# sthagen/foundationdb

Hardware: AMD Instinct MI355X
Metric: resolved txns/sec (conflict ranges checked/sec) per batch; HBM GB/s vs peak (higher is better)
Workload: dtype u8/int64 (byte keys, int64 versions)

## Files before the change

### foundationdb_amd/csrc/engine.cpp

```cpp
#include <hip/hip_runtime.h>
#include <stdio.h>
#include <stdlib.h>
#include <string.h>
#include <unistd.h>

#include <cxxabi.h>

#include <algorithm>
#include <array>
#include <atomic>
#include <chrono>
#include <condition_variable>
#include <functional>
#include <mutex>
#include <new>
#include <string>
#include <thread>
#include <unordered_set>
#include <vector>

#include "../../include/fdb_conflict_set.h"
#include "engine.h"

using namespace fdbcs;
// ... 482 lines not shown
    for (int pass = 0; pass < 2; pass++) {
    if (pass == 1) {
        if (int rc = cs->ws[k][0].ensure(align_up(off, (size_t)2 << 20))) return rc;
        arena = (char*)cs->ws[k][0].p;
        off = 0;
    }
#define TAKE(field, bytes) \
    if (int rc = take((bytes), (void**)&w.field)) return rc
    TAKE(hist_conf, T);
    TAKE(rconf, R);
    TAKE(status, T);
    TAKE(first_conf, 4 * T);
    const int64_t slab_buckets = std::min<int64_t>(kSortMaxBuckets, (E + kSortTarget - 1) / kSortTarget + 1);
    TAKE(items, sizeof(SortItem) * E);
    TAKE(scnt, 8 * kCntStride * (size_t)kSortMaxBuckets);
    TAKE(slab, sizeof(SortItem) * kSlab * slab_buckets);
    TAKE(ovf, sizeof(SortItem) * E);
    TAKE(ovf_b, 4 * E);
    TAKE(big, sizeof(SortItem) * E);
    TAKE(big_p, 4 * E);
    TAKE(samples, sizeof(SortItem) * kMaxSample);
    TAKE(srank, 4 * (kMaxSample + 64));
    w.slab_buckets = (int32_t)slab_buckets;
    TAKE(pos, 4 * E);
    TAKE(pmeta, 4 * E);
    TAKE(cwb, 4 * (E + 1));
    TAKE(crb, 4 * (E + 1));
    TAKE(cwe, 4 * (E + 1));
    TAKE(wends, 8 * (2 * W + 1));
    TAKE(wkeys, sizeof(DKey) * (2 * W + 1));
    TAKE(segk, sizeof(DKey) * (2 * W + 2));
    TAKE(cflag, 2 * W + 2);
    TAKE(wbrange, 4 * W);
    TAKE(wlead, 4 * (W + 1));
    TAKE(wtxn, 4 * (W + 1));
    TAKE(gminc, 4 * (W + 1));
    TAKE(rbrange, 4 * R);
    TAKE(eoff, 4 * (R + 1));
    TAKE(poff, 4 * (R + W + 1));
    TAKE(pcg, 4 * (R + W + 1));
    TAKE(pcoff, 4 * (R + W + 1));
    TAKE(pcbase, 4 * (R + W + 1));
    TAKE(pca, 4 * (R + W + 1));
    TAKE(ecur, 4 * R);
    TAKE(edges, 4 * edge_cap);
    TAKE(eptr, 4 * T);
    TAKE(pre_st, T);
    TAKE(pre_ep, 4 * T);
    TAKE(pre_end, 4 * T);
    TAKE(ulist, 32 * T);
    TAKE(wpk, 4 * (W + 1));
    TAKE(tedges, 4 * edge_cap);
    TAKE(mcs_bits, 8 * (E / 64 + 2));
    TAKE(seg_b, 4 * (W + 1));
    TAKE(seg_e, 4 * (W + 1));
    TAKE(seg_lo, 8 * (W + 1));
    TAKE(seg_hi, 8 * (W + 1));
    TAKE(seg_rem, 8 * (W + 1));
    TAKE(seg_ins, 8 * (W + 1));
    TAKE(seg_tlen, 8 * (W + 1));
    TAKE(seg_endins, W + 1);
    TAKE(seg_vend, 8 * (W + 1));
    TAKE(verdict, T);
    TAKE(bsc, sizeof(BatchScalars));
    }
#undef TAKE
    w.edge_cap = edge_cap;
    w.cap_T = T;
    w.cap_R = R;
    HIPOK(hipMemsetAsync(w.hist_conf, 0, T, cs->stream));
    HIPOK(hipMemsetAsync(w.rconf, 0, R, cs->stream));
    HIPOK(hipMemsetAsync(w.ecur, 0, 4 * R, cs->stream));
    HIPOK(hipMemsetAsync(w.scnt, 0, 8 * kCntStride * (size_t)kSortMaxBuckets, cs->stream));
    HIPOK(hipMemsetAsync(w.srank, 0, 4 * (kMaxSample + 64), cs->stream));
    HIPOK(hipMemsetAsync(w.bsc, 0, sizeof(BatchScalars), cs->stream));
    if (k >= 1) {
        Work& w0 = cs->work[0];
        w.c_lo = w0.c_lo, w.c_hi = w0.c_hi, w.c_rem = w0.c_rem, w.c_ins = w0.c_ins, w.c_val = w0.c_val;
// ... 3079 lines not shown
```

### foundationdb_amd/csrc/engine.h

```cpp
#pragma once
#include <hip/hip_runtime.h>
#include <stdint.h>
#include <limits.h>

#include "dkey.h"
#include "scan.h"

namespace fdbcs {

constexpr int kBlock = 256;
constexpr int kWG = 1024;
constexpr int kSortTile = 4096;
constexpr int kFan = 64;
constexpr int kMaxLevels = 4;
constexpr int kL3Rep = 8;
constexpr int kL3Pad = 16;
__host__ __device__ constexpr int64_t l3_words(int64_t n) { return n * kL3Rep * kL3Pad; }
constexpr int kGcTile = 4096;
constexpr int kMaxGroupWrites = 12288;
constexpr int kMaxTxnLds = 49152;

enum : uint8_t { kUndecided = 0, kAborted = 1, kCommitted = 2 };
enum : uint8_t { kFlagTooOld = 1, kFlagReport = 2 };

// ... 60 lines not shown
    int32_t debug_error;
    int32_t ovf_n;
    int32_t sort_big;
    int64_t n_segments;
    int64_t n_pranges;
    int32_t n_undec;
    int32_t pad2;
};

constexpr int64_t kHole = INT64_MIN;

struct TierIO {
    const int64_t* n_in;
    int64_t* n_out;
    int64_t* before;
    int64_t* removed;
};

struct Segs {
    int64_t *lo, *hi, *rem, *ins;
    int32_t* tile_first;
};

enum ScanKind { kScanEdges, kScanSegSum, kScanCompact, kScanGc, kScanCover, kScanSegNum, kScanFold, kNumScans };

struct BatchDev {
    int32_t T, R, W;
    int64_t* snap;
    uint8_t* flags;
    int32_t* roff;
    int32_t* woff;
    int32_t* rowner;
    int32_t* wowner;
    DKey* keys;
    uint8_t* tail;
    int64_t tail_n;
};

#ifndef FDBCS_SORT_TARGET
#define FDBCS_SORT_TARGET 64
#endif
constexpr int kSortTarget = FDBCS_SORT_TARGET;
constexpr int kSlab = 256;
constexpr int kSortMaxBuckets = 4096;
constexpr int kQuant = 4096;
constexpr int kQuantMinE = 2048;
constexpr int kMaxSample = 8192;
// ... 3 lines not shown
constexpr int kCntStride = FDBCS_CNT_STRIDE;
constexpr int kSplitWords = 8;
constexpr int kSplitBytes = 8 * kSplitWords;
struct SplitKey {
    uint64_t w[kSplitWords];
    uint32_t len, meta;
};

struct Work {
    uint8_t* hist_conf;
    uint8_t* rconf;
    uint8_t* status;
    int32_t* first_conf;
    SortItem* items;
    uint64_t* scnt;
    SortItem* slab;
    int32_t slab_buckets;
    SortItem* ovf;
    int32_t* ovf_b;
    SortItem* big;
    int32_t* big_p;
    SortItem* samples;
    int32_t* srank;
    int32_t* pos;
    uint32_t* pmeta;
    int32_t* cwb;
    int32_t* crb;
    int32_t* cwe;
    int2* wends;
    DKey* wkeys;
    DKey* segk;
    uint8_t* cflag;
    uint8_t* btail;
    int32_t* wbrange;
    int32_t* rbrange;
    int32_t* eoff;
    int32_t* poff;
    int32_t* pcg;
    int32_t* pcoff;
    int32_t* pcbase;
    int32_t* pca;
    int32_t* ecur;
    int32_t* wlead;
    int32_t* wtxn;
    int32_t* gminc;
    int32_t groups = 0;
    int32_t* edges;
    int64_t edge_cap;
    int32_t* eptr;
    uint8_t* pre_st;
    int32_t* pre_ep;
    int32_t* pre_end;
    int4* ulist;
    uint32_t* wpk;
    int32_t report = 0;
    int32_t* tedges;
    uint64_t* mcs_bits;
    int32_t* seg_b;
    int32_t* seg_e;
    int64_t* seg_lo;
    int64_t* seg_hi;
    int64_t* seg_rem;
    int64_t* seg_ins;
    int64_t* seg_tlen;
    uint8_t* seg_endins;
    int64_t* seg_vend;
    uint8_t* verdict;
    BatchScalars* bsc;
    ScanState scan[kNumScans];
    int64_t scan_gran[kNumScans];
    uint64_t* scan_arena;
    int64_t scan_words;
    int64_t cap_T, cap_R;
    int32_t* tile_first;
    int64_t *c_lo, *c_hi, *c_rem, *c_ins, *c_val;
    uint8_t* c_exact;
    unsigned long long* trace;
    int32_t no_prepass;
    uint32_t* hedge;
    uint32_t hseq;
    uint8_t* vdev;
};
// ... 270 lines not shown
```

### foundationdb_amd/csrc/kernels.hip

```cpp
#include <hip/hip_runtime.h>
#include <stdio.h>
#include <stdlib.h>
#include <algorithm>
#include <vector>
#include <limits.h>

#include "engine.h"
#include "lane_xor.h"

namespace fdbcs {

thread_local LaunchList* t_record = nullptr;
thread_local uint8_t t_group = 0;
thread_local hipError_t t_launch_error = hipSuccess;


__device__ __forceinline__ const uint8_t* hist_tail(const uint8_t* htail, uint32_t unit) {
    return htail + 8 * (size_t)unit;
}
__device__ __forceinline__ uint32_t tail_units(uint32_t len) { return len > 16u ? (len - 16u + 7u) / 8u : 0u; }

__device__ __forceinline__ void copy_tail_words(uint8_t* dst, const uint8_t* src, uint32_t n) {
    const uintptr_t a = (uintptr_t)src;
    const uint64_t* w = (const uint64_t*)(a & ~(uintptr_t)7);
// ... 1215 lines not shown
    const uint32_t slot = (uint32_t)old;
    if (slot < (uint32_t)kSlab) {
        a.slab[(size_t)bk * kSlab + slot] = it;
    } else {
        const int o = atomicAdd(&a.bsc->ovf_n, 1);
        a.ovf[o] = it;
        a.ovf_b[o] = bk;
    }
    if (a.trace) {
        asm volatile("s_waitcnt vmcnt(0)" ::: "memory");
        trace_max(a.trace, kTrPartEnd);
        if ((threadIdx.x & 63) == 0) {
            const unsigned long long tp4 = wall_clock64();
            atomicAdd(&a.trace[kTrPartWaves], 1ull);
            atomicAdd(&a.trace[kTrPartSumFill], tp1 - tp0);
            atomicAdd(&a.trace[kTrPartSumCopy], tp2 - tp1);
            atomicAdd(&a.trace[kTrPartSumSearch], tp3 - tp2);
            atomicAdd(&a.trace[kTrPartSumPlace], tp4 - tp3);
        }
    }
}

struct SortOut {
    int32_t* pos;
    uint32_t* pmeta;
    int32_t *cwb, *crb, *cwe;
    int32_t *wbrange, *rbrange;
    SortItem* items;
    SplitKey* quant;
    SortItem* big;
    int32_t* big_p;
};

template <int S>
__device__ __forceinline__ void wave_bitonic(uint64_t (&kh)[4], uint64_t (&kl)[4], uint64_t (&ka)[4]) {
    const int lane = threadIdx.x & 63;
#pragma unroll
    for (int k = 2; k <= 64 * S; k <<= 1) {
#pragma unroll
        for (int j = k >> 1; j > 0; j >>= 1) {
            if (j >= 64) {
                const int js = j >> 6;
#pragma unroll
                for (int s = 0; s < S; s++) {
                    if (s & js) continue;
                    const int t = s | js;
                    const bool up = ((s * 64 + lane) & k) == 0;
                    if (key3_less(kh[t], kl[t], ka[t], kh[s], kl[s], ka[s]) == up) {
                        uint64_t x = kh[s]; kh[s] = kh[t]; kh[t] = x;
// ... 18 lines not shown
        }
    }
}

__device__ __forceinline__ uint32_t endpoint_meta(const BatchDev& b, int p) {
    const int g = p >> 1, e = p & 1;
    const uint32_t cls = g < b.R ? (e ? kReadEnd : kReadBegin) : (e ? kWriteEnd : kWriteBegin);
    return ((uint32_t)g << 3) | ((uint32_t)e << 2) | cls;
}

__device__ __forceinline__ void put_quantiles(const BatchDev& b, SplitKey* quant, int64_t P, int64_t E, int p) {
    int q = (int)((P * (kQuant + 1) + E - 1) / E) - 1;
    if (q < 0) q = 0;
    if (q >= kQuant || quant_pos(q, E) > P) return;
    const SplitKey sk = make_split(make_item(b, p), b.tail);
    for (; q < kQuant && quant_pos(q, E) <= P; q++)
        if (quant_pos(q, E) == P) quant[q] = sk;
}

__device__ __forceinline__ void put_position(const BatchDev& b, const SortOut& o, int p, int64_t P, int32_t wb,
                                             int32_t rb, int32_t we) {
    const uint32_t meta = endpoint_meta(b, p);
    const uint32_t cls = item_class(meta);
    o.pmeta[P] = meta;
    o.pos[p] = (int32_t)P;
    o.cwb[P] = wb;
    o.crb[P] = rb;
    o.cwe[P] = we;
    if (cls == kWriteBegin) o.wbrange[wb] = p >> 1;
    if (cls == kReadBegin) o.rbrange[rb] = p >> 1;
    if (o.items) o.items[P] = make_item(b, p);
}

__device__ __forceinline__ uint32_t split_lcp(const SplitKey& a, const SplitKey& b) {
    uint32_t c = 0;
#pragma unroll
    for (int i = 0; i < kSplitWords; i++) {
        const uint64_t x = a.w[i] ^ b.w[i];
        if (x) {
            c = 8 * i + (uint32_t)(__builtin_clzll(x) >> 3);
            break;
        }
        c = 8 * (i + 1);
    }
    c = c < a.len ? c : a.len;
    return c < b.len ? c : b.len;
}

template <bool LONG>
__global__ __launch_bounds__(kBlock) void k_sort_bucket(BatchDev b, SortArgs a, SortOut o) {
    constexpr int kWaves = kBlock / 64;
// ... 262 lines not shown
        if (lane == 0) {
#pragma unroll
            for (int c = 0; c < 4; c++) {
                s_red[c][wave] = pre[c];
                s_red[4 + c][wave] = tot[c];
            }
            const uint32_t v[4] = {(uint32_t)own0, (uint32_t)(own0 >> 32), (uint32_t)own1, (uint32_t)(own1 >> 32)};
#pragma unroll
            for (int c = 0; c < 4; c++) s_cnt[wave][c] = v[c];
            s_big[wave] = n > kSlab ? 1 : 0;
        }
        __syncthreads();
        if (threadIdx.x == 0) {
            uint32_t run[4] = {0, 0, 0, 0};
            for (int q = 0; q < kWaves; q++)
#pragma unroll
                for (int c = 0; c < 4; c++) run[c] += s_red[c][q];
            for (int q = 0; q < kWaves; q++)
#pragma unroll
                for (int c = 0; c < 4; c++) {
                    s_base[q][c] = run[c];
                    run[c] += s_cnt[q][c];
                }
            if (blockIdx.x == 0) {
                uint32_t t4[4] = {0, 0, 0, 0};
                for (int q = 0; q < kWaves; q++)
#pragma unroll
                    for (int c = 0; c < 4; c++) t4[c] += s_red[4 + c][q];
                o.cwb[E] = (int32_t)t4[1];
                o.crb[E] = (int32_t)t4[2];
                o.cwe[E] = (int32_t)t4[3];
            }
        }
        __syncthreads();
        if (threadIdx.x == 0) trace_max(a.trace, kTrBktPrologue);
    }
    if (small) {
        const int64_t base = s_base[wave][0];
        const unsigned long long tw3 = a.trace ? wall_clock64() : 0ull;
        uint32_t carry[3] = {s_base[wave][1], s_base[wave][2], s_base[wave][3]};
#pragma unroll
        for (int s = 0; s < 4; s++) {
            if (s >= S) break;
            const int k = s * 64 + lane;
            const bool live = k < n;
            const uint32_t cls = live ? item_class(endpoint_meta(b, ps[s])) : 4u;
            const uint32_t f[3] = {cls == kWriteBegin, cls == kReadBegin, cls == kWriteEnd};
            uint32_t ex[3];
#pragma unroll
            for (int q = 0; q < 3; q++) {
                uint32_t x = f[q];
#pragma unroll
                for (int off = 1; off < 64; off <<= 1) {
                    const uint32_t y = __shfl_up(x, off, 64);
                    if (lane >= off) x += y;
                }
                ex[q] = carry[q] + x - f[q];
                carry[q] += __shfl(x, 63, 64);
            }
            if (live && !(a.exp & 2)) {
                put_position(b, o, ps[s], base + k, (int32_t)ex[0], (int32_t)ex[1], (int32_t)ex[2]);
                if (o.quant) put_quantiles(b, o.quant, base + k, E, ps[s]);
            } else if (live && ex[0] == 0x7fffffff) {
                o.pos[0] = 0;
            }
        }
        if (a.trace && lane == 0) {
            asm volatile("s_waitcnt vmcnt(0)" ::: "memory");
            const unsigned long long tw4 = wall_clock64();
            atomicAdd(&a.trace[kTrBktWaves], 1ull);
            atomicAdd(&a.trace[kTrBktSumLoad], tt[1] - tt[0]);
            atomicAdd(&a.trace[kTrBktSumSort], tt[2] - tt[1]);
            atomicAdd(&a.trace[kTrBktSumTies], tw3 - tt[2]);
            atomicAdd(&a.trace[kTrBktSumPut], tw4 - tw3);
        }
    }
    __syncthreads();
    for (int wv = 0; wv < kWaves; wv++) {
        if (!s_big[wv] || B0 + wv >= nb) continue;
        const int bb = B0 + wv;
        const int m = (int)s_cnt[wv][0];
        const int64_t bbase = s_base[wv][0];
        if (threadIdx.x == 0) {
            s_gather = 0;
            atomicAdd(&a.bsc->sort_big, 1);
        }
        for (int i = threadIdx.x; i < kSlab; i += kBlock) o.big[bbase + i] = a.slab[(size_t)bb * kSlab + i];
// ... 71 lines not shown
    a.long_keys = long_keys ? 1 : 0;
    return a;
}

void launch_sort(hipStream_t s, const BatchDev& b, const Work& w, SplitKey* quant, SplitKey* quant_out, bool cold,
                 int bucket_target, bool long_keys, bool validate, hipEvent_t sort_begin, hipEvent_t sort_end) {
    const int E = 2 * (b.R + b.W);
    if (E == 0) return;
    const int nb = sort_bucket_count(E, bucket_target, w.slab_buckets);
    fdb_event(LaunchList::kTimingRecord, sort_begin, s);
    if (cold && nb > 1) {
        SampleRank c{};
        c.S = sort_cold_samples(E, nb);
        c.n_slice = (c.S + kSampleSlice - 1) / kSampleSlice;
        c.srank = w.srank;
        c.samples = w.samples;
        c.trace = w.trace;
        fdb_launch(k_sample, dim3(c.n_slice * ((c.S + kBlock - 1) / kBlock)), dim3(kBlock), 0, s, b, c);
        fdb_launch(k_quant_cold, dim3(1), dim3(kWG), 0, s, b, (const SortItem*)w.samples, (const int32_t*)w.srank,
                   c.S, quant);
    }
    const SortArgs a = sort_args(w, quant, nb, b.tail_n, long_keys);
    fdb_launch(k_sort_partition, dim3((E + kBlock - 1) / kBlock), dim3(kBlock), (uint32_t)(16 * (nb - 1)), s, b, a);
    SortOut o{w.pos, w.pmeta, w.cwb, w.crb, w.cwe, w.wbrange, w.rbrange, validate ? w.items : nullptr,
              quant_out, w.big, w.big_p};
    const int grid = (nb + kBlock / 64 - 1) / (kBlock / 64);
    if (long_keys)
        fdb_launch(k_sort_bucket<true>, dim3(grid), dim3(kBlock), 0, s, b, a, o);
    else
        fdb_launch(k_sort_bucket<false>, dim3(grid), dim3(kBlock), 0, s, b, a, o);
    fdb_event(LaunchList::kTimingRecord, sort_end, s);
}

hipError_t debug_time_sort(hipStream_t s, const BatchDev& b, const Work& w, SplitKey* quant, int bucket_target,
                           bool long_keys, int which, int reps, double* us) {
    const int E = 2 * (b.R + b.W);
    if (E == 0) return hipErrorInvalidValue;
    const int nb = sort_bucket_count(E, bucket_target, w.slab_buckets);
    hipEvent_t e0, e1;
    hipError_t err;
    if ((err = hipEventCreate(&e0)) || (err = hipEventCreate(&e1))) return err;
    SortArgs a = sort_args(w, quant, nb, b.tail_n, long_keys);
    if (const char* v = getenv("FDBCS_SORT_EXP")) a.exp = atoi(v);
    SortOut o{w.pos, w.pmeta, w.cwb, w.crb, w.cwe, w.wbrange, w.rbrange, nullptr, nullptr, w.big, w.big_p};
    const int grid = (nb + kBlock / 64 - 1) / (kBlock / 64);
    double total = 0;
    for (int r = 0; r < reps && err == hipSuccess; r++) {
        (void)hipMemsetAsync(w.scnt, 0, 8 * kCntStride * (size_t)kSortMaxBuckets, s);
        (void)hipMemsetAsync(&w.bsc->ovf_n, 0, 4, s);
        if (which == 1) (void)hipEventRecord(e0, s);
        fdb_launch(k_sort_partition, dim3((E + kBlock - 1) / kBlock), dim3(kBlock), (uint32_t)(16 * (nb - 1)), s, b, a);
        if (which == 1) (void)hipEventRecord(e1, s);
        if (which == 2) (void)hipEventRecord(e0, s);
        if (long_keys)
            fdb_launch(k_sort_bucket<true>, dim3(grid), dim3(kBlock), 0, s, b, a, o);
        else
            fdb_launch(k_sort_bucket<false>, dim3(grid), dim3(kBlock), 0, s, b, a, o);
        if (which == 2) (void)hipEventRecord(e1, s);
        if ((err = hipEventSynchronize(e1))) break;
        float ms = 0;
        if ((err = hipEventElapsedTime(&ms, e0, e1))) break;
        total += ms;
    }
    (void)hipMemsetAsync(w.scnt, 0, 8 * kCntStride * (size_t)kSortMaxBuckets, s);
    (void)hipMemsetAsync(w.bsc, 0, sizeof(BatchScalars), s);
    (void)hipStreamSynchronize(s);
    (void)hipEventDestroy(e0);
    (void)hipEventDestroy(e1);
    *us = total * 1000.0 / reps;
    return err;
}

__global__ __launch_bounds__(kBlock) void k_validate_sort(const SortItem* sorted, const int32_t* pos,
                                                          const uint32_t* pmeta, int E, const uint8_t* arena,
                                                          BatchScalars* sc) {
    const int p = blockIdx.x * blockDim.x + threadIdx.x;
    if (p >= E) return;
    bool bad = p > 0 && !item_less_total(sorted[p - 1], sorted[p], arena);
    bad |= sorted[p].meta != pmeta[p];
    const int q = pos[p];
    bad |= q < 0 || q >= E || (2 * item_range(pmeta[q]) + item_is_end(pmeta[q])) != (uint32_t)p;
    if (bad) atomicOr(&sc->debug_error, 1);
}

void launch_validate_sort(hipStream_t s, const BatchDev& b, const Work& w) {
    const int E = 2 * (b.R + b.W);
    if (E == 0) return;
    fdb_launch(k_validate_sort, dim3((E + kBlock - 1) / kBlock), dim3(kBlock), 0, s, (const SortItem*)w.items,
               (const int32_t*)w.pos, (const uint32_t*)w.pmeta, E, (const uint8_t*)b.tail, w.bsc);
}



__device__ __forceinline__ bool range_nonempty(const Work& w, int g) { return w.pos[2 * g] < w.pos[2 * g + 1]; }

__device__ __forceinline__ uint2 write_rb_interval(const Work& w, int g) {
    const int b = w.pos[2 * g], e = w.pos[2 * g + 1];
    if (b >= e) return make_uint2(0, 0);
    const int lo = w.crb[b], hi = w.crb[e];
    return hi > lo ? make_uint2((uint32_t)lo, (uint32_t)hi) : make_uint2(0, 0);
}

constexpr int kEdgeScanP = 1;
constexpr int kCombineP = 1;
constexpr int kCombineTile = kScanThreads * kCombineP;
constexpr int kRouteScanP = 1;

struct EdgePairScan {
    Work w;
    int32_t R, G;
    const int32_t* wowner;
    const DKey* keys;
    const int32_t* rowner;
    int32_t T;
    __device__ void counts(int64_t g, uint32_t& slots, uint32_t& pairs, uint32_t& a) const {
        slots = pairs = a = 0;
        if (g >= R) {
            const int pb = w.pos[2 * g], pe = w.pos[2 * g + 1];
            const int code = pb < pe ? 2 * wowner[g - R] : -1;
            const int ib = w.cwb[pb] + w.cwe[pb], ie = w.cwb[pe] + w.cwe[pe];
            w.wends[ib] = make_int2(pb, code);
            w.wends[ie] = make_int2(pe, code < 0 ? -1 : code + 1);
            w.wkeys[ib] = keys[2 * g];
            w.wkeys[ie] = keys[2 * g + 1];
        }
        if (g >= R && w.groups) {
            const int j = w.cwb[w.pos[2 * g]];
            const uint2 iv = write_rb_interval(w, (int)g);
            int lead = 0;
            if (iv.y > iv.x) {
                lead = 2;
                if (j > 0) {
                    const int gp = w.wbrange[j - 1];
                    const uint2 ip = write_rb_interval(w, gp);
                    if (ip.x == iv.x && ip.y == iv.y) lead = 1;
                }
            }
            w.wlead[j] = lead;
            w.wtxn[j] = wowner[g - R];
            if (lead == 2) pairs = iv.y - iv.x;
            return;
        }
        if (!range_nonempty(w, (int)g)) return;
        const int b = w.pos[2 * g], e = w.pos[2 * g + 1];
        if (g < R) {
            a = (uint32_t)(w.cwb[e] - w.cwb[b]);
            const int cover = w.cwb[b] - w.cwe[b];
            slots = a + (uint32_t)(cover > 0 ? cover : 0);
            pairs = a;
        } else {
            pairs = (uint32_t)(w.crb[e] - w.crb[b]);
        }
    }
    static constexpr bool kOwn = true;
    __device__ void load(int64_t g, uint32_t (&v)[3]) const {
        uint32_t a;
        counts(g, v[0], v[1], a);
        v[2] = v[1] > 0 ? 1u : 0u;
    }
    __device__ void store(int64_t g, const uint32_t (&ex)[3], const uint32_t (&own)[3]) const {
        if (g < R) w.eoff[g] = (int32_t)ex[0];
        w.poff[g] = (int32_t)ex[1];
        if (own[2]) {
            w.pcg[ex[2]] = (int32_t)g;
            w.pcoff[ex[2]] = (int32_t)ex[1];
            const int p0 = w.pos[2 * g];
            if (g < R) {
                w.pcbase[ex[2]] = w.cwb[p0];
                w.pca[ex[2]] = rowner[g];
            } else {
                w.pcbase[ex[2]] = w.crb[p0];
                w.pca[ex[2]] = w.groups ? T + w.cwb[p0] : wowner[g - R];
            }
        }
    }
    __device__ void finish(const uint32_t (&tot)[3]) const {
        w.eoff[R] = (int32_t)tot[0];
        w.poff[G] = (int32_t)tot[1];
        w.pcg[tot[2]] = G;
        w.pcoff[tot[2]] = (int32_t)tot[1];
        w.bsc->n_pranges = tot[2];
        w.bsc->n_edges = tot[0];
        w.bsc->edge_overflow = (int64_t)tot[0] > w.edge_cap || tot[0] > 0x7fffffffu || tot[1] > 0x7fffffffu ? 1 : 0;
        if (w.hedge) {
            w.hedge[1] = tot[0] != 0 ? 1u : 0u;
            __threadfence_system();
            w.hedge[0] = w.hseq;
        }
    }
};

constexpr int kPairsPerThread = 4;
constexpr int kFillPairs = kBlock * kPairsPerThread;

__device__ __forceinline__ int wave_last_le(const int32_t* a, int lo, int hi, int x) {
// ... 118 lines not shown
    BatchDev b;
    int use_status;
    __device__ int delta(int64_t i) const {
        const int2 e = w.wends[i];
        if (e.y < 0) return 0;
        const int t = e.y >> 1;
        const bool committed = use_status ? w.status[t] == kCommitted
                                          : (!w.hist_conf[t] && !(b.flags[t] & kFlagTooOld));
        return committed ? ((e.y & 1) ? -1 : 1) : 0;
    }
    __device__ void load(int64_t i, uint32_t (&v)[1]) const { v[0] = (uint32_t)delta(i); }
    __device__ void store(int64_t i, const uint32_t (&ex)[1]) const {
        const int d = delta(i), c = (int)ex[0];
        w.cflag[i] = (d == 1 && c == 0) ? 1 : ((d == -1 && c == 1) ? 2 : 0);
    }
    __device__ void finish(const uint32_t (&)[1]) const {}
};
struct SegNumScan {
    Work w;
    __device__ void load(int64_t i, uint32_t (&v)[1]) const { v[0] = w.cflag[i] == 1 ? 1u : 0u; }
    __device__ void store(int64_t i, const uint32_t (&ex)[1]) const {
        const uint8_t f = w.cflag[i];
        if (!f) return;
        const int x = w.wends[i].x;
        if (f == 1) {
            w.seg_b[ex[0]] = x;
            w.segk[2 * ex[0]] = w.wkeys[i];
        } else {
            w.seg_e[ex[0] - 1] = x;
            w.segk[2 * ex[0] - 1] = w.wkeys[i];
        }
    }
    __device__ void finish(const uint32_t (&tot)[1]) const { w.bsc->n_segments = tot[0]; }
};

__global__ __launch_bounds__(kBlock) void k_resolve_pre(BatchDev b, Work w, uint8_t* vout) {
    const BatchScalars* sc = w.bsc;
    const int T = b.T;
    if (blockIdx.x == 0 && threadIdx.x == 0) trace_min(w.trace, kTrResBegin);
    if (sc->n_edges == 0 && !sc->edge_overflow) {
        if (blockIdx.x == 0 && threadIdx.x == 0) w.bsc->rounds = 0;
        for (int t = blockIdx.x * blockDim.x + threadIdx.x; t < T; t += gridDim.x * blockDim.x) {
            const uint8_t st = (w.hist_conf[t] || (b.flags[t] & kFlagTooOld)) ? kAborted : kCommitted;
            w.status[t] = st;
            w.first_conf[t] = INT_MAX;
            vout[t] = verdict_byte(b, t, st);
            if (w.vdev) w.vdev[t] = vout[t];
        }
        __shared__ uint32_t sv[1][scan_pad(kCombineP)];
        __shared__ uint32_t swave[1][kScanThreads / 64];
        __shared__ uint32_t sbase[1];
        __shared__ int s_tile;
        const int64_t n = 2 * (int64_t)b.W;
        const int64_t ntiles = n > 0 ? (n + kCombineTile - 1) / kCombineTile : 1;
// ... 376 lines not shown
                    if (p < s1) break;
                }
                if (r == rend) res = kCommitted;
                w.eptr[t] = p;
                if (res != kUndecided)
                    vst[t] = res;
                else
                    more = 1;
            }
            if (more) s_more = 1;
            __syncthreads();
            rounds++;
            if (!s_more) break;
            __syncthreads();
        }
    } else {
        const int E = 2 * (b.R + b.W);
        for (int i = threadIdx.x; i <= E / 64; i += blockDim.x) w.mcs_bits[i] = 0;
        __syncthreads();
        for (int t = 0; t < T; t++) {
            if (st[t] != kUndecided) continue;
            int conflict_at = INT_MAX;
            for (int r = b.roff[t]; r < b.roff[t + 1]; r++) {
                const int a = w.pos[2 * r], e = w.pos[2 * r + 1];
                int hit = 0;
                if (a < e) {
                    for (int word = (a >> 6) + threadIdx.x; word <= ((e - 1) >> 6); word += blockDim.x) {
                        uint64_t m = ((volatile uint64_t*)w.mcs_bits)[word];
                        const int lo = word << 6;
                        if (a > lo) m &= ~0ull << (a - lo);
                        if (e < lo + 64) m &= (e - lo >= 64) ? ~0ull : ((1ull << (e - lo)) - 1);
                        if (m) hit = 1;
                    }
                }
                if (__syncthreads_or(hit)) {
                    conflict_at = r - b.roff[t];
                    break;
                }
            }
            if (conflict_at == INT_MAX) {
                for (int x = b.woff[t]; x < b.woff[t + 1]; x++) {
                    const int g = b.R + x;
                    const int a = w.pos[2 * g], e = w.pos[2 * g + 1];
                    if (a < e) {
                        for (int word = (a >> 6) + threadIdx.x; word <= ((e - 1) >> 6); word += blockDim.x) {
                            uint64_t m = ~0ull;
                            const int lo = word << 6;
                            if (a > lo) m &= ~0ull << (a - lo);
                            if (e < lo + 64) m &= (e - lo >= 64) ? ~0ull : ((1ull << (e - lo)) - 1);
                            atomicOr((unsigned long long*)&w.mcs_bits[word], (unsigned long long)m);
                        }
                    }
                    __syncthreads();
                }
            }
            if (threadIdx.x == 0) {
                st[t] = conflict_at == INT_MAX ? kCommitted : kAborted;
                if (conflict_at != INT_MAX) w.first_conf[t] = conflict_at;
            }
            __syncthreads();
        }
        rounds = -1;
    }
    __syncthreads();
    if (threadIdx.x == 0) trace_max(w.trace, kTrResRounds);
    if (NW && !overflow && w.report) {
// ... 84 lines not shown
struct Epilogue {
    uint8_t* verdict_out;
    uint32_t* flag;
    uint32_t seq;
    unsigned long long* trace;
    int32_t T;
    int compacted, gc_ran;
    uint8_t* zero8;
    int64_t zero8_n;
    uint8_t* zero8r;
    int64_t zero8r_n;
    int32_t* zero32b;
    int64_t zero32_n;
    uint64_t* zero64[kNumScans + 1];
    int64_t zero64_n[kNumScans + 1];
    uint64_t* zero_bc;
    int64_t zero_bc_n;
    int32_t* zero_rank;
    int64_t zero_rank_n;
    BatchScalars* bsc;
    int64_t* nd_out;
};


__device__ __forceinline__ const DKey& seg_key(const BatchDev& b, const Work& w, int pos, int end) {
    const int g = (int)item_range(w.pmeta[pos]);
    return b.keys[2 * g + end];
}

constexpr int kDeltaTile = 256;
constexpr int kBaseTile = 4096;

__device__ __forceinline__ void fill_tile_first(int32_t* tile_first, const int64_t* lo, int64_t j, int tile) {
    const int64_t t0 = j > 0 ? lo[j - 1] / tile + 1 : 0;
    for (int64_t t = t0; t <= lo[j] / tile; t++) tile_first[t] = (int32_t)j;
}
__device__ __forceinline__ void fill_tile_first_tail(int32_t* tile_first, const int64_t* lo, int64_t U, int64_t n,
                                                     int tile) {
    const int64_t t0 = U > 0 ? lo[U - 1] / tile + 1 : 0;
    for (int64_t t = t0; t <= n / tile + 1; t++) tile_first[t] = (int32_t)U;
}

constexpr int kSegWideMinW = 24576;
constexpr int seg_per(bool long_keys, bool wide) { return long_keys || !wide ? 63 : 127; }
constexpr int seg_lanes(bool, bool wide) { return wide ? 1 : kArity; }
constexpr int seg_threads(bool long_keys, bool wide) {
    return 2 * seg_lanes(long_keys, wide) * (seg_per(long_keys, wide) + 1);
}
inline bool seg_wide(int64_t W, bool long_keys) { return long_keys || W >= kSegWideMinW; }
inline int64_t seg_tiles(int64_t W, bool long_keys, bool wide) { return (W > 0 ? W : 1) / seg_per(long_keys, wide) + 1; }
inline int64_t seg_prep_tiles(int64_t W) { return (W > 0 ? W : 1) / 63 + 1; }
// ... 7 lines not shown
    constexpr int LL = seg_lanes(LONG, WIDE);
    constexpr int NSW = (SP + 1 + 63) / 64;
    __shared__ int64_t s_lo[SP + 1];
    __shared__ uint32_t s_val[3][SP + 1];
    __shared__ uint32_t s_wsum[3][NSW];
    __shared__ uint32_t s_base[3];
    __shared__ int s_tile;
    const int64_t gt = (int64_t)blockIdx.x * blockDim.x + threadIdx.x;
    for (int64_t i = gt; i < lvl3_n * kL3Rep; i += (int64_t)gridDim.x * blockDim.x) lvl3[i * kL3Pad] = LLONG_MIN;
    for (int64_t i = gt; i < lvl2_n; i += (int64_t)gridDim.x * blockDim.x) lvl2[i] = LLONG_MIN;
    if (threadIdx.x == 0) s_tile = atomicAdd(w.scan[kScanSegSum].counter, 1);
    __syncthreads();
    const int tile = s_tile;
    const int U = (int)w.bsc->n_segments;
    const int ntiles = U > 0 ? (U + SP - 1) / SP : 1;
    if (tile >= ntiles) return;
    const int64_t n = *io.n_in;
    const int q = threadIdx.x / (2 * LL), role = (threadIdx.x / LL) & 1;
    const int sg = tile * SP + (q < SP ? q : -1);
    const bool live = sg >= 0 && sg < U && (q < SP || role == 0);
    int64_t pos = 0;
    bool eq = false;
    DKey kb{}, ke{};
    if (live) {
        kb = seg_key(b, w, w.seg_b[sg], 0);
        ke = seg_key(b, w, w.seg_e[sg], 1);
        const DKey& key = role ? ke : kb;
        if constexpr (LONG) {
            static_assert(WIDE, "long-key batches take the one-lane layout");
            QTail qt;
            load_qtail(qt, key, b.tail);
            pos = lane_lower_bound_long(h, hm, n, key, qt, htail, b.tail, eq);
        } else if constexpr (WIDE) {
            pos = lane_lower_bound(h, hm, n, key, htail, b.tail, eq);
        } else {
            pos = group_lower_bound<false>(h, hm, n, key, htail, b.tail, eq);
        }
    }
    const int lane = threadIdx.x & 63, wid = threadIdx.x >> 6;
    const int64_t hi = __shfl(pos, (lane + LL) & 63, 64);
    const int exact = __shfl((int)eq, (lane + LL) & 63, 64);
    if (threadIdx.x % (2 * LL) == 0) {
        if (q == SP) {
            s_lo[0] = live ? pos : 0;
        } else if (live) {
            const int64_t lo = pos;
            const bool glue = sg + 1 < U && dkey_cmp(seg_key(b, w, w.seg_b[sg + 1], 0), b.tail, ke, b.tail) == 0;
            const bool endins = !exact && !glue;
            w.seg_lo[sg] = lo;
            w.seg_hi[sg] = hi;
            w.seg_endins[sg] = endins ? 1 : 0;
            w.seg_vend[sg] = hi > 0 ? h.ver[hi - 1] : kHole;
            s_lo[q + 1] = lo;
            s_val[0][q] = (uint32_t)(hi - lo);
            s_val[1][q] = endins ? 2 : 1;
            s_val[2][q] = tail_units(kb.len) + (endins ? tail_units(ke.len) : 0u);
        } else {
            s_val[0][q] = s_val[1][q] = s_val[2][q] = 0;
        }
    }
    __syncthreads();
    uint32_t ex[3] = {0, 0, 0};
    if (wid < NSW) {
#pragma unroll
        for (int c = 0; c < 3; c++) {
            const uint32_t v = threadIdx.x < SP ? s_val[c][threadIdx.x] : 0u;
            uint32_t x = v;
#pragma unroll
            for (int o = 1; o < 64; o <<= 1) {
                const uint32_t y = __shfl_up(x, o, 64);
// ... 131 lines not shown
        } else {
            for (int64_t i = i0 + threadIdx.x; i < i1; i += blockDim.x) {
                int64_t lo = 0, hi = U;
                while (lo < hi) {
                    int64_t mid = (lo + hi) >> 1;
                    if (g.lo[mid] <= i) lo = mid + 1; else hi = mid;
                }
                const int64_t j = lo - 1;
                if (j >= 0 && i >= g.lo[j] && i < g.hi[j]) continue;
                const int64_t o = i + g.ins[j + 1] - g.rem[j + 1];
                dst.key[o] = src.key[i];
                dst.lt[o] = src.lt[i];
                dst.ver[o] = src.ver[i];
            }
        }
        __syncthreads();
    }
    for (int64_t sg = (int64_t)blockIdx.x * blockDim.x + threadIdx.x; sg < U; sg += (int64_t)gridDim.x * blockDim.x)
        ins((int)sg, dst, g.lo[sg] - g.rem[sg] + g.ins[sg]);
}

struct BatchIns {
    BatchDev b;
    const uint32_t* pmeta;
    const int32_t *seg_b, *seg_e;
    const int64_t *tlen, *vend;
    const uint8_t* endins;
    uint8_t* htail;
    const Scalars* sc;
    int64_t now;
    __device__ const DKey& key(int pos, int end) const {
        return b.keys[2 * (int)item_range(pmeta[pos]) + end];
    }
    __device__ void operator()(int s, Hist dst, int64_t o) const {
        int64_t tu = sc->tail_used / 8 + tlen[s];
        const DKey kb = key(seg_b[s], 0);
        uint32_t tb = 0;
        if (kb.len > 16) {
            tb = (uint32_t)tu;
            copy_tail_words(htail + 8 * tu, b.tail + kb.tail, kb.len - 16);
            tu += tail_units(kb.len);
        }
        dst.key[o] = make_ulonglong2(kb.hi, kb.lo);
        dst.lt[o] = make_uint2(kb.len, tb);
        dst.ver[o] = now;
        if (endins[s]) {
            const DKey ke = key(seg_e[s], 1);
            uint32_t te = 0;
            if (ke.len > 16) {
                te = (uint32_t)tu;
                copy_tail_words(htail + 8 * tu, b.tail + ke.tail, ke.len - 16);
            }
            dst.key[o + 1] = make_ulonglong2(ke.hi, ke.lo);
            dst.lt[o + 1] = make_uint2(ke.len, te);
            dst.ver[o + 1] = vend[s];
        }
    }
};

static Segs batch_segs(const Work& w) { return Segs{w.seg_lo, w.seg_hi, w.seg_rem, w.seg_ins, w.tile_first}; }

static unsigned copy_tiles(int64_t grid_hint_n, int tile, int64_t max_inserts = 0) {
    int64_t tiles = (grid_hint_n + 1 + tile - 1) / tile;
    tiles = std::max<int64_t>(tiles, (max_inserts + kBlock - 1) / kBlock);
    if (tiles < 1) tiles = 1;
    if (tiles > 8192) tiles = 8192;
    return (unsigned)tiles;
}

static Epilogue make_epilogue(const BatchDev& b, const Work& w, int compacted, int gc_ran, uint8_t* verdict_out,
// ... 23 lines not shown
        ep.zero64[k + 1] = w.scan[k].granules;
        ep.zero64_n[k + 1] = std::min<int64_t>(used[k], w.scan_gran[k]);
    }
    ep.zero_bc = w.scnt;
    ep.zero_bc_n = sort_nb;
    ep.zero_rank = w.srank;
    ep.zero_rank_n = sort_samples;
    ep.bsc = w.bsc;
    return ep;
}

void launch_merge(hipStream_t s, const BatchDev& b, const Work& w, const Hist& src, const MaxLevels& srcm,
                  const Hist& dst, const MaxLevels& dstm, const int64_t* nd_src, uint8_t* htail, Scalars* sc,
                  int64_t now, int64_t lvl3_n, int64_t lvl2_n, int64_t grid_hint_n, hipEvent_t copy_begin,
                  hipEvent_t copy_end, bool long_keys) {
    const TierIO io{nd_src, &sc->nd_next, &sc->d_before, &sc->d_rem};
    const bool wide = seg_wide(b.W, long_keys);
    fdb_launch(long_keys ? k_seg_prep<true, true> : (wide ? k_seg_prep<false, true> : k_seg_prep<false, false>),
               dim3((unsigned)seg_tiles(b.W, long_keys, wide)), dim3(seg_threads(long_keys, wide)), 0, s, b, w, src, srcm, htail, sc, io, dstm.lvl[3], lvl3_n,
               dstm.lvl[2], lvl2_n);
    fdb_event(LaunchList::kTimingRecord, copy_begin, s);
    BatchIns ins{};
    ins.b = b;
    ins.pmeta = w.pmeta;
    ins.seg_b = w.seg_b;
    ins.seg_e = w.seg_e;
    ins.tlen = w.seg_tlen;
    ins.vend = w.seg_vend;
    ins.endins = w.seg_endins;
    ins.htail = htail;
    ins.sc = sc;
    ins.now = now;
    fdb_launch((k_merge_copy<BatchIns, kDeltaTile>), dim3(copy_tiles(grid_hint_n, kDeltaTile, b.W)), dim3(kBlock), 0,
               s, batch_segs(w), src, dst, nd_src, &w.bsc->n_segments, ins);
    fdb_event(LaunchList::kTimingRecord, copy_end, s);
}


template <int MODE>
__global__ __launch_bounds__(kBlock) void k_compact_search(Hist base, MaxLevels basem, Hist delta,
                                                           const uint8_t* htail, const int64_t* nb_ptr,
                                                           const int64_t* nd_ptr, int64_t hdr, Work w, int64_t* lvl3,
                                                           int64_t lvl3_n, int64_t* lvl2, int64_t lvl2_n) {
    const int64_t gt = (int64_t)blockIdx.x * blockDim.x + threadIdx.x;
    for (int64_t i = gt; i < lvl3_n * kL3Rep; i += (int64_t)gridDim.x * blockDim.x) lvl3[i * kL3Pad] = LLONG_MIN;
    for (int64_t i = gt; i < lvl2_n; i += (int64_t)gridDim.x * blockDim.x) lvl2[i] = LLONG_MIN;
    const int64_t j = gt;
    const int64_t nd = *nd_ptr;
    if (j >= nd) return;
// ... 1522 lines not shown
```

Baseline: 54.21 million.

## Pack per-endpoint sort outputs into one int4 record and read segment keys directly

Replaces the separate pos/pmeta/cwb/crb/cwe arrays with a single int4 record per endpoint, written in one store and indexed by original endpoint rather than sorted position. Edge counting, segment prep and merge copy now read that packed record, or read segk directly, instead of chasing the pos→pmeta→keys indirections. This drops the seg_b/seg_e arrays and a scan kind. The aim is fewer scattered global loads and stores. The cost is that cumulative counts are now read at the endpoint's own index rather than at sorted positions, which changes their semantics and needs a consistent producer.

```diff
diff --git a/foundationdb_amd/csrc/engine.cpp b/foundationdb_amd/csrc/engine.cpp
--- a/foundationdb_amd/csrc/engine.cpp
+++ b/foundationdb_amd/csrc/engine.cpp
@@ -528,11 +528,7 @@
     TAKE(samples, sizeof(SortItem) * kMaxSample);
     TAKE(srank, 4 * (kMaxSample + 64));
     w.slab_buckets = (int32_t)slab_buckets;
-    TAKE(pos, 4 * E);
-    TAKE(pmeta, 4 * E);
-    TAKE(cwb, 4 * (E + 1));
-    TAKE(crb, 4 * (E + 1));
-    TAKE(cwe, 4 * (E + 1));
+    TAKE(erec, sizeof(int4) * E);
     TAKE(wends, 8 * (2 * W + 1));
     TAKE(wkeys, sizeof(DKey) * (2 * W + 1));
     TAKE(segk, sizeof(DKey) * (2 * W + 2));
@@ -558,8 +554,6 @@
     TAKE(wpk, 4 * (W + 1));
     TAKE(tedges, 4 * edge_cap);
     TAKE(mcs_bits, 8 * (E / 64 + 2));
-    TAKE(seg_b, 4 * (W + 1));
-    TAKE(seg_e, 4 * (W + 1));
     TAKE(seg_lo, 8 * (W + 1));
     TAKE(seg_hi, 8 * (W + 1));
     TAKE(seg_rem, 8 * (W + 1));
diff --git a/foundationdb_amd/csrc/engine.h b/foundationdb_amd/csrc/engine.h
--- a/foundationdb_amd/csrc/engine.h
+++ b/foundationdb_amd/csrc/engine.h
@@ -106,7 +106,7 @@
     int32_t* tile_first;
 };
 
-enum ScanKind { kScanEdges, kScanSegSum, kScanCompact, kScanGc, kScanCover, kScanSegNum, kScanFold, kNumScans };
+enum ScanKind { kScanEdges, kScanSegSum, kScanCompact, kScanGc, kScanCover, kScanSegNum, kNumScans };
 
 struct BatchDev {
     int32_t T, R, W;
@@ -156,11 +156,7 @@
     int32_t* big_p;
     SortItem* samples;
     int32_t* srank;
-    int32_t* pos;
-    uint32_t* pmeta;
-    int32_t* cwb;
-    int32_t* crb;
-    int32_t* cwe;
+    int4* erec;
     int2* wends;
     DKey* wkeys;
     DKey* segk;
@@ -190,8 +186,6 @@
     int32_t report = 0;
     int32_t* tedges;
     uint64_t* mcs_bits;
-    int32_t* seg_b;
-    int32_t* seg_e;
     int64_t* seg_lo;
     int64_t* seg_hi;
     int64_t* seg_rem;
diff --git a/foundationdb_amd/csrc/kernels.hip b/foundationdb_amd/csrc/kernels.hip
--- a/foundationdb_amd/csrc/kernels.hip
+++ b/foundationdb_amd/csrc/kernels.hip
@@ -1261,9 +1261,7 @@
 }
 
 struct SortOut {
-    int32_t* pos;
-    uint32_t* pmeta;
-    int32_t *cwb, *crb, *cwe;
+    int4* erec;
     int32_t *wbrange, *rbrange;
     SortItem* items;
     SplitKey* quant;
@@ -1328,11 +1326,7 @@
                                              int32_t rb, int32_t we) {
     const uint32_t meta = endpoint_meta(b, p);
     const uint32_t cls = item_class(meta);
-    o.pmeta[P] = meta;
-    o.pos[p] = (int32_t)P;
-    o.cwb[P] = wb;
-    o.crb[P] = rb;
-    o.cwe[P] = we;
+    o.erec[p] = make_int4((int32_t)P, wb, rb, we);
     if (cls == kWriteBegin) o.wbrange[wb] = p >> 1;
     if (cls == kReadBegin) o.rbrange[rb] = p >> 1;
     if (o.items) o.items[P] = make_item(b, p);
@@ -1641,15 +1635,6 @@
                     s_base[q][c] = run[c];
                     run[c] += s_cnt[q][c];
                 }
-            if (blockIdx.x == 0) {
-                uint32_t t4[4] = {0, 0, 0, 0};
-                for (int q = 0; q < kWaves; q++)
-#pragma unroll
-                    for (int c = 0; c < 4; c++) t4[c] += s_red[4 + c][q];
-                o.cwb[E] = (int32_t)t4[1];
-                o.crb[E] = (int32_t)t4[2];
-                o.cwe[E] = (int32_t)t4[3];
-            }
         }
         __syncthreads();
         if (threadIdx.x == 0) trace_max(a.trace, kTrBktPrologue);
@@ -1681,7 +1666,7 @@
                 put_position(b, o, ps[s], base + k, (int32_t)ex[0], (int32_t)ex[1], (int32_t)ex[2]);
                 if (o.quant) put_quantiles(b, o.quant, base + k, E, ps[s]);
             } else if (live && ex[0] == 0x7fffffff) {
-                o.pos[0] = 0;
+                o.erec[0] = make_int4(0, 0, 0, 0);
             }
         }
         if (a.trace && lane == 0) {
@@ -1799,7 +1784,7 @@
     }
     const SortArgs a = sort_args(w, quant, nb, b.tail_n, long_keys);
     fdb_launch(k_sort_partition, dim3((E + kBlock - 1) / kBlock), dim3(kBlock), (uint32_t)(16 * (nb - 1)), s, b, a);
-    SortOut o{w.pos, w.pmeta, w.cwb, w.crb, w.cwe, w.wbrange, w.rbrange, validate ? w.items : nullptr,
+    SortOut o{w.erec, w.wbrange, w.rbrange, validate ? w.items : nullptr,
               quant_out, w.big, w.big_p};
     const int grid = (nb + kBlock / 64 - 1) / (kBlock / 64);
     if (long_keys)
@@ -1819,7 +1804,7 @@
     if ((err = hipEventCreate(&e0)) || (err = hipEventCreate(&e1))) return err;
     SortArgs a = sort_args(w, quant, nb, b.tail_n, long_keys);
     if (const char* v = getenv("FDBCS_SORT_EXP")) a.exp = atoi(v);
-    SortOut o{w.pos, w.pmeta, w.cwb, w.crb, w.cwe, w.wbrange, w.rbrange, nullptr, nullptr, w.big, w.big_p};
+    SortOut o{w.erec, w.wbrange, w.rbrange, nullptr, nullptr, w.big, w.big_p};
     const int grid = (nb + kBlock / 64 - 1) / (kBlock / 64);
     double total = 0;
     for (int r = 0; r < reps && err == hipSuccess; r++) {
@@ -1848,15 +1833,17 @@
     return err;
 }
 
-__global__ __launch_bounds__(kBlock) void k_validate_sort(const SortItem* sorted, const int32_t* pos,
-                                                          const uint32_t* pmeta, int E, const uint8_t* arena,
-                                                          BatchScalars* sc) {
+__global__ __launch_bounds__(kBlock) void k_validate_sort(const SortItem* sorted, const int4* erec, int E,
+                                                          const uint8_t* arena, BatchScalars* sc) {
     const int p = blockIdx.x * blockDim.x + threadIdx.x;
     if (p >= E) return;
     bool bad = p > 0 && !item_less_total(sorted[p - 1], sorted[p], arena);
-    bad |= sorted[p].meta != pmeta[p];
-    const int q = pos[p];
-    bad |= q < 0 || q >= E || (2 * item_range(pmeta[q]) + item_is_end(pmeta[q])) != (uint32_t)p;
+    const int q = erec[p].x;
+    bad |= q < 0 || q >= E;
+    if (!bad) {
+        const uint32_t m = sorted[q].meta;
+        bad = (2 * item_range(m) + item_is_end(m)) != (uint32_t)p;
+    }
     if (bad) atomicOr(&sc->debug_error, 1);
 }
 
@@ -1864,18 +1851,18 @@
     const int E = 2 * (b.R + b.W);
     if (E == 0) return;
     fdb_launch(k_validate_sort, dim3((E + kBlock - 1) / kBlock), dim3(kBlock), 0, s, (const SortItem*)w.items,
-               (const int32_t*)w.pos, (const uint32_t*)w.pmeta, E, (const uint8_t*)b.tail, w.bsc);
-}
-
-
-
-__device__ __forceinline__ bool range_nonempty(const Work& w, int g) { return w.pos[2 * g] < w.pos[2 * g + 1]; }
-
-__device__ __forceinline__ uint2 write_rb_interval(const Work& w, int g) {
-    const int b = w.pos[2 * g], e = w.pos[2 * g + 1];
-    if (b >= e) return make_uint2(0, 0);
-    const int lo = w.crb[b], hi = w.crb[e];
-    return hi > lo ? make_uint2((uint32_t)lo, (uint32_t)hi) : make_uint2(0, 0);
+               (const int4*)w.erec, E, (const uint8_t*)b.tail, w.bsc);
+}
+
+
+
+__device__ __forceinline__ bool range_nonempty(const Work& w, int g) {
+    return w.erec[2 * g].x < w.erec[2 * g + 1].x;
+}
+
+__device__ __forceinline__ uint2 write_rb_interval(const int4& rb, const int4& re) {
+    if (rb.x >= re.x) return make_uint2(0, 0);
+    return re.z > rb.z ? make_uint2((uint32_t)rb.z, (uint32_t)re.z) : make_uint2(0, 0);
 }
 
 constexpr int kEdgeScanP = 1;
@@ -1890,50 +1877,52 @@
     const DKey* keys;
     const int32_t* rowner;
     int32_t T;
-    __device__ void counts(int64_t g, uint32_t& slots, uint32_t& pairs, uint32_t& a) const {
-        slots = pairs = a = 0;
-        if (g >= R) {
-            const int pb = w.pos[2 * g], pe = w.pos[2 * g + 1];
-            const int code = pb < pe ? 2 * wowner[g - R] : -1;
-            const int ib = w.cwb[pb] + w.cwe[pb], ie = w.cwb[pe] + w.cwe[pe];
-            w.wends[ib] = make_int2(pb, code);
-            w.wends[ie] = make_int2(pe, code < 0 ? -1 : code + 1);
-            w.wkeys[ib] = keys[2 * g];
-            w.wkeys[ie] = keys[2 * g + 1];
-        }
-        if (g >= R && w.groups) {
-            const int j = w.cwb[w.pos[2 * g]];
-            const uint2 iv = write_rb_interval(w, (int)g);
-            int lead = 0;
-            if (iv.y > iv.x) {
-                lead = 2;
-                if (j > 0) {
-                    const int gp = w.wbrange[j - 1];
-                    const uint2 ip = write_rb_interval(w, gp);
-                    if (ip.x == iv.x && ip.y == iv.y) lead = 1;
-                }
-            }
-            w.wlead[j] = lead;
-            w.wtxn[j] = wowner[g - R];
-            if (lead == 2) pairs = iv.y - iv.x;
-            return;
-        }
-        if (!range_nonempty(w, (int)g)) return;
-        const int b = w.pos[2 * g], e = w.pos[2 * g + 1];
-        if (g < R) {
-            a = (uint32_t)(w.cwb[e] - w.cwb[b]);
-            const int cover = w.cwb[b] - w.cwe[b];
-            slots = a + (uint32_t)(cover > 0 ? cover : 0);
-            pairs = a;
-        } else {
-            pairs = (uint32_t)(w.crb[e] - w.crb[b]);
-        }
-    }
     static constexpr bool kOwn = true;
     __device__ void load(int64_t g, uint32_t (&v)[3]) const {
-        uint32_t a;
-        counts(g, v[0], v[1], a);
-        v[2] = v[1] > 0 ? 1u : 0u;
+        const int4* __restrict__ erec = w.erec;
+        const int32_t* __restrict__ wbrange = w.wbrange;
+        const int32_t* __restrict__ wown = wowner;
+        const DKey* __restrict__ k = keys;
+        const int4 rb = erec[2 * g], re = erec[2 * g + 1];
+        const bool nonempty = rb.x < re.x;
+        uint32_t slots = 0, pairs = 0;
+        if (g < R) {
+            if (nonempty) {
+                const uint32_t a = (uint32_t)(re.y - rb.y);
+                const int cover = rb.y - rb.w;
+                slots = a + (uint32_t)(cover > 0 ? cover : 0);
+                pairs = a;
+            }
+        } else {
+            const int own = wown[g - R];
+            const int code = nonempty ? 2 * own : -1;
+            const int ib = rb.y + rb.w, ie = re.y + re.w;
+            w.wends[ib] = make_int2(rb.x, code);
+            w.wends[ie] = make_int2(re.x, code < 0 ? -1 : code + 1);
+            w.wkeys[ib] = k[2 * g];
+            w.wkeys[ie] = k[2 * g + 1];
+            if (w.groups) {
+                const int j = rb.y;
+                const uint2 iv = write_rb_interval(rb, re);
+                int lead = 0;
+                if (iv.y > iv.x) {
+                    lead = 2;
+                    if (j > 0) {
+                        const int gp = wbrange[j - 1];
+                        const uint2 ip = write_rb_interval(erec[2 * gp], erec[2 * gp + 1]);
+                        if (ip.x == iv.x && ip.y == iv.y) lead = 1;
+                    }
+                }
+                w.wlead[j] = lead;
+                w.wtxn[j] = own;
+                if (lead == 2) pairs = iv.y - iv.x;
+            } else if (nonempty) {
+                pairs = (uint32_t)(re.z - rb.z);
+            }
+        }
+        v[0] = slots;
+        v[1] = pairs;
+        v[2] = pairs > 0 ? 1u : 0u;
     }
     __device__ void store(int64_t g, const uint32_t (&ex)[3], const uint32_t (&own)[3]) const {
         if (g < R) w.eoff[g] = (int32_t)ex[0];
@@ -1941,13 +1930,13 @@
         if (own[2]) {
             w.pcg[ex[2]] = (int32_t)g;
             w.pcoff[ex[2]] = (int32_t)ex[1];
-            const int p0 = w.pos[2 * g];
+            const int4 rb = w.erec[2 * g];
             if (g < R) {
-                w.pcbase[ex[2]] = w.cwb[p0];
+                w.pcbase[ex[2]] = rb.y;
                 w.pca[ex[2]] = rowner[g];
             } else {
-                w.pcbase[ex[2]] = w.crb[p0];
-                w.pca[ex[2]] = w.groups ? T + w.cwb[p0] : wowner[g - R];
+                w.pcbase[ex[2]] = rb.z;
+                w.pca[ex[2]] = w.groups ? T + rb.y : wowner[g - R];
             }
         }
     }
@@ -2112,14 +2101,8 @@
     __device__ void store(int64_t i, const uint32_t (&ex)[1]) const {
         const uint8_t f = w.cflag[i];
         if (!f) return;
-        const int x = w.wends[i].x;
-        if (f == 1) {
-            w.seg_b[ex[0]] = x;
-            w.segk[2 * ex[0]] = w.wkeys[i];
-        } else {
-            w.seg_e[ex[0] - 1] = x;
-            w.segk[2 * ex[0] - 1] = w.wkeys[i];
-        }
+        if (f == 1) w.segk[2 * ex[0]] = w.wkeys[i];
+        else w.segk[2 * ex[0] - 1] = w.wkeys[i];
     }
     __device__ void finish(const uint32_t (&tot)[1]) const { w.bsc->n_segments = tot[0]; }
 };
@@ -2542,7 +2525,7 @@
             if (st[t] != kUndecided) continue;
             int conflict_at = INT_MAX;
             for (int r = b.roff[t]; r < b.roff[t + 1]; r++) {
-                const int a = w.pos[2 * r], e = w.pos[2 * r + 1];
+                const int a = w.erec[2 * r].x, e = w.erec[2 * r + 1].x;
                 int hit = 0;
                 if (a < e) {
                     for (int word = (a >> 6) + threadIdx.x; word <= ((e - 1) >> 6); word += blockDim.x) {
@@ -2561,7 +2544,7 @@
             if (conflict_at == INT_MAX) {
                 for (int x = b.woff[t]; x < b.woff[t + 1]; x++) {
                     const int g = b.R + x;
-                    const int a = w.pos[2 * g], e = w.pos[2 * g + 1];
+                    const int a = w.erec[2 * g].x, e = w.erec[2 * g + 1].x;
                     if (a < e) {
                         for (int word = (a >> 6) + threadIdx.x; word <= ((e - 1) >> 6); word += blockDim.x) {
                             uint64_t m = ~0ull;
@@ -2692,11 +2675,6 @@
     int64_t* nd_out;
 };
 
-
-__device__ __forceinline__ const DKey& seg_key(const BatchDev& b, const Work& w, int pos, int end) {
-    const int g = (int)item_range(w.pmeta[pos]);
-    return b.keys[2 * g + end];
-}
 
 constexpr int kDeltaTile = 256;
 constexpr int kBaseTile = 4096;
@@ -2750,9 +2728,10 @@
     int64_t pos = 0;
     bool eq = false;
     DKey kb{}, ke{};
+    const DKey* __restrict__ segk = w.segk;
     if (live) {
-        kb = seg_key(b, w, w.seg_b[sg], 0);
-        ke = seg_key(b, w, w.seg_e[sg], 1);
+        kb = segk[2 * sg];
+        ke = segk[2 * sg + 1];
         const DKey& key = role ? ke : kb;
         if constexpr (LONG) {
             static_assert(WIDE, "long-key batches take the one-lane layout");
@@ -2773,7 +2752,7 @@
             s_lo[0] = live ? pos : 0;
         } else if (live) {
             const int64_t lo = pos;
-            const bool glue = sg + 1 < U && dkey_cmp(seg_key(b, w, w.seg_b[sg + 1], 0), b.tail, ke, b.tail) == 0;
+            const bool glue = sg + 1 < U && dkey_cmp(segk[2 * (sg + 1)], b.tail, ke, b.tail) == 0;
             const bool endins = !exact && !glue;
             w.seg_lo[sg] = lo;
             w.seg_hi[sg] = hi;
@@ -2951,19 +2930,15 @@
 
 struct BatchIns {
     BatchDev b;
-    const uint32_t* pmeta;
-    const int32_t *seg_b, *seg_e;
+    const DKey* segk;
     const int64_t *tlen, *vend;
     const uint8_t* endins;
     uint8_t* htail;
     const Scalars* sc;
     int64_t now;
-    __device__ const DKey& key(int pos, int end) const {
-        return b.keys[2 * (int)item_range(pmeta[pos]) + end];
-    }
     __device__ void operator()(int s, Hist dst, int64_t o) const {
         int64_t tu = sc->tail_used / 8 + tlen[s];
-        const DKey kb = key(seg_b[s], 0);
+        const DKey kb = segk[2 * s];
         uint32_t tb = 0;
         if (kb.len > 16) {
             tb = (uint32_t)tu;
@@ -2974,7 +2949,7 @@
         dst.lt[o] = make_uint2(kb.len, tb);
         dst.ver[o] = now;
         if (endins[s]) {
-            const DKey ke = key(seg_e[s], 1);
+            const DKey ke = segk[2 * s + 1];
             uint32_t te = 0;
             if (ke.len > 16) {
                 te = (uint32_t)tu;
@@ -3044,9 +3019,7 @@
     fdb_event(LaunchList::kTimingRecord, copy_begin, s);
     BatchIns ins{};
     ins.b = b;
-    ins.pmeta = w.pmeta;
-    ins.seg_b = w.seg_b;
-    ins.seg_e = w.seg_e;
+    ins.segk = w.segk;
     ins.tlen = w.seg_tlen;
     ins.vend = w.seg_vend;
     ins.endins = w.seg_endins;
```

After: 55.66 million, median of 6. +2.7%, better.
